# Aceinna/gnss-ins-sim

Hardware: AMD Instinct MI355X
Metric: Monte-Carlo IMU samples integrated/sec (higher is better)
Workload: dtype f64

## Files before the change

### gnss-ins-sim_amd/csrc/ginsim_api.hip

```cpp
#include <hip/hip_runtime.h>
#include <chrono>

#include <cmath>
#include <cstdarg>
#include <cstdio>
#include <cstring>
#include <string>
#include <vector>

#include "ginsim.h"
#include "allan.hpp"
#include "comm.hpp"
#include "launch.hpp"
#include "placed.hpp"

namespace ginsim {

static thread_local std::string g_err;

void set_error(const char* fmt, ...) {
    char buf[512];
    va_list ap;
    va_start(ap, fmt);
    vsnprintf(buf, sizeof(buf), fmt, ap);
    va_end(ap);
    g_err = buf;
}

}

using namespace ginsim;

struct ginsim_ctx {
    int device;
    hipStream_t stream;
    hipEvent_t ev0, ev1;
    std::vector<hipEvent_t> pool;
    void* ws[4] = {nullptr, nullptr, nullptr, nullptr};
    size_t ws_bytes[4] = {0, 0, 0, 0};
    double* allan_host = nullptr;
    size_t allan_host_doubles = 0;
    ginsim::Comm* comm = nullptr;
    double* comm_recv = nullptr;
    ginsim_stats* comm_host = nullptr;
    hipEvent_t comm_ev[8] = {};
    bool comm_pending[8] = {};
    ginsim_stats* stat_slots = nullptr;
    hipEvent_t stat_ev[8] = {};
    bool stat_pending[8] = {};
    unsigned long long* selftest = nullptr;
};

static hipError_t scratch(ginsim_ctx* c, int slot, size_t bytes, void** out) {
    if (c->ws_bytes[slot] < bytes) {
        if (c->ws[slot]) {
            hipError_t e = hipStreamSynchronize(c->stream);
            if (e != hipSuccess) return e;
            e = hipFree(c->ws[slot]);
            if (e != hipSuccess) return e;
            c->ws[slot] = nullptr;
            c->ws_bytes[slot] = 0;
        }
        const size_t want = bytes + bytes / 4 + 4096;
        hipError_t e = hipMalloc(&c->ws[slot], want);
        if (e != hipSuccess) return e;
        c->ws_bytes[slot] = want;
    }
    *out = c->ws[slot];
    return hipSuccess;
}

#define HIP_TRY(expr)                                                                         \
    do {                                                                                      \
        hipError_t e_ = (expr);                                                               \
        if (e_ != hipSuccess) {                                                               \
            set_error("%s failed: %s (%s:%d)", #expr, hipGetErrorString(e_), __FILE__, __LINE__); \
            if (e_ == hipErrorOutOfMemory) { (void)hipGetLastError(); return GINSIM_ERR_NOMEM; } \
            return GINSIM_ERR_HIP;                                                            \
        }                                                                                     \
    } while (0)
// ... 17 lines not shown

int ginsim_abi_version(void) { return GINSIM_ABI_VERSION; }

const char* ginsim_last_error(void) { return g_err.c_str(); }

int ginsim_device_count(int* count) {
    REQUIRE(count, "device_count: NULL output");
    int n = 0;
    const hipError_t e = hipGetDeviceCount(&n);
    if (e != hipSuccess) {
        *count = 0;
        set_error("hipGetDeviceCount: %s", hipGetErrorString(e));
        return GINSIM_ERR_NODEV;
    }
    *count = n;
    return GINSIM_OK;
}

int ginsim_create(int device, ginsim_ctx** out) {
    REQUIRE(out, "create: NULL output");
    *out = nullptr;
    int n = 0;
    if (hipGetDeviceCount(&n) != hipSuccess || n < 1) {
        set_error("no HIP device visible (the engine has no CPU fallback)");
        return GINSIM_ERR_NODEV;
    }
    REQUIRE(device >= 0 && device < n, "create: device %d out of range [0,%d)", device, n);
    HIP_TRY(hipSetDevice(device));
    ginsim_ctx* c = new ginsim_ctx();
    c->device = device;
    HIP_TRY(hipStreamCreateWithFlags(&c->stream, hipStreamNonBlocking));
    HIP_TRY(hipEventCreate(&c->ev0));
    HIP_TRY(hipEventCreate(&c->ev1));
    ginsim::placed_context_created(device);
    *out = c;
    return GINSIM_OK;
}

int ginsim_destroy(ginsim_ctx* c) {
    if (!c) return GINSIM_OK;
    (void)hipSetDevice(c->device);
    (void)hipStreamSynchronize(c->stream);
    (void)hipEventDestroy(c->ev0);
    (void)hipEventDestroy(c->ev1);
    for (hipEvent_t e : c->pool)
        if (e) (void)hipEventDestroy(e);
    for (void* w : c->ws)
        if (w) (void)hipFree(w);
    for (hipEvent_t e : c->stat_ev)
        if (e) (void)hipEventDestroy(e);
    if (c->stat_slots) (void)hipHostFree(c->stat_slots);
    if (c->allan_host) (void)hipHostFree(c->allan_host);
    if (c->selftest) (void)hipFree(c->selftest);
    if (c->comm) ginsim::comm_destroy(c->comm);
    if (c->comm_recv) (void)hipFree(c->comm_recv);
    if (c->comm_host) (void)hipHostFree(c->comm_host);
    for (hipEvent_t e : c->comm_ev)
        if (e) (void)hipEventDestroy(e);
    ginsim::vib_psd_drop_plans(c->stream);
    (void)hipStreamDestroy(c->stream);
    ginsim::placed_free_owner(c->device, c);
    ginsim::placed_context_destroyed(c->device);
    delete c;
    return GINSIM_OK;
}

int ginsim_device_name(ginsim_ctx* c, char* buf, size_t cap) {
    REQUIRE(c && buf && cap > 0, "device_name: bad arguments");
    hipDeviceProp_t prop;
    HIP_TRY(hipGetDeviceProperties(&prop, c->device));
    snprintf(buf, cap, "%s (%s, %d CUs)", prop.name, prop.gcnArchName, prop.multiProcessorCount);
    return GINSIM_OK;
}

int ginsim_malloc(ginsim_ctx* c, size_t bytes, void** dptr) {
    REQUIRE(c && dptr, "malloc: bad arguments");
    HIP_TRY(hipSetDevice(c->device));
    HIP_TRY(hipMalloc(dptr, bytes ? bytes : 8));
    return GINSIM_OK;
}

int ginsim_placed_configure(ginsim_ctx* c, const ginsim_placed_options* o) {
    REQUIRE(c && o, "placed_configure: bad arguments");
    return ginsim::placed_configure(c->device, *o);
// ... 463 lines not shown
}

extern "C" {

int ginsim_aux_sensors(ginsim_ctx* c, const ginsim_aux_params* p) {
    REQUIRE(c && p, "aux_sensors: NULL argument");
    REQUIRE(p->runs >= 1 && p->n >= 0 && p->m >= 0, "aux_sensors: bad sizes");
    REQUIRE(!p->out_gps || p->ref_gps, "aux_sensors: ref_gps missing");
    REQUIRE(!p->out_mag || p->ref_mag, "aux_sensors: ref_mag missing");
    REQUIRE(p->n <= 0xFFFFFFFFll && p->m <= 0xFFFFFFFFll, "aux_sensors: sample index exceeds the RNG counter");
    REQUIRE((double)p->n * (double)p->runs < 5.0e11 && (double)p->m * (double)p->runs < 5.0e11, "aux_sensors: too many elements");
    HIP_TRY(hipSetDevice(c->device));
    HIP_TRY(launch_aux(*p, c->stream));
    return GINSIM_OK;
}

int ginsim_magcal_run(ginsim_ctx* c, const ginsim_magcal_params* p) {
    REQUIRE(c && p, "magcal_run: NULL argument");
    REQUIRE(p->runs >= 1, "magcal_run: runs=%lld must be >= 1", (long long)p->runs);
    REQUIRE(p->n >= 1 && p->n <= 0xFFFFFFFFll, "magcal_run: n must lie in 1 .. the 32-bit sample counter of the RNG");
    REQUIRE(p->runs <= (int64_t)0x7FFFFFFF * 64, "magcal_run: too many runs for one launch");
    REQUIRE(p->in_mag || p->ref_mag, "magcal_run: neither ref_mag (generated form) nor in_mag (given form)");
    REQUIRE(p->out_si && p->out_hi, "magcal_run: out_si / out_hi missing");
    for (int a = 0; a < 3; ++a) {
        const long long s0 = (long long)p->seg[2 * a], s1 = (long long)p->seg[2 * a + 1];
        REQUIRE(s0 >= 0 && s1 <= (long long)p->n, "magcal_run: range %c [%lld, %lld) is outside [0, %lld]", "xyz"[a], s0, s1, (long long)p->n);
        REQUIRE(s0 < s1, "magcal_run: range %c [%lld, %lld) is empty", "xyz"[a], s0, s1);
    }
    HIP_TRY(hipSetDevice(c->device));
    HIP_TRY(launch_magcal(*p, c->stream));
    return GINSIM_OK;
}

int ginsim_end_stats(ginsim_ctx* c, const double* end_err, int64_t runs, ginsim_stats* host_out) {
    REQUIRE(c && end_err && host_out && runs >= 1, "end_stats: bad arguments");
    HIP_TRY(hipSetDevice(c->device));
    void* ws = nullptr;
    HIP_TRY(scratch(c, 0, stats_scratch_bytes(runs), &ws));
    HIP_TRY(launch_end_stats(end_err, runs, ws, c->stream));
    const char* res = reinterpret_cast<char*>(ws) + stats_scratch_bytes(runs) - sizeof(ginsim_stats);
    HIP_TRY(hipMemcpyAsync(host_out, res, sizeof(ginsim_stats), hipMemcpyDeviceToHost, c->stream));
    HIP_TRY(hipStreamSynchronize(c->stream));
    return GINSIM_OK;
}

int ginsim_end_stats_begin(ginsim_ctx* c, const double* end_err, int64_t runs, int32_t slot) {
    REQUIRE(c && end_err && runs >= 1 && slot >= 0 && slot < 8, "end_stats_begin: bad arguments");
    REQUIRE(!c->stat_pending[slot], "end_stats_begin: slot %d is still pending (call ginsim_end_stats_finish first)", slot);
    HIP_TRY(hipSetDevice(c->device));
    if (!c->stat_slots) HIP_TRY(hipHostMalloc(reinterpret_cast<void**>(&c->stat_slots), 8 * sizeof(ginsim_stats), hipHostMallocDefault));
    if (!c->stat_ev[slot]) HIP_TRY(hipEventCreateWithFlags(&c->stat_ev[slot], hipEventDisableTiming));
    void* ws = nullptr;
    HIP_TRY(scratch(c, 0, stats_scratch_bytes(runs), &ws));
    HIP_TRY(launch_end_stats(end_err, runs, ws, c->stream));
    const char* res = reinterpret_cast<char*>(ws) + stats_scratch_bytes(runs) - sizeof(ginsim_stats);
    HIP_TRY(hipMemcpyAsync(&c->stat_slots[slot], res, sizeof(ginsim_stats), hipMemcpyDeviceToHost, c->stream));
    HIP_TRY(hipEventRecord(c->stat_ev[slot], c->stream));
    c->stat_pending[slot] = true;
    return GINSIM_OK;
}

int ginsim_end_stats_finish(ginsim_ctx* c, int32_t slot, ginsim_stats* host_out) {
    REQUIRE(c && host_out && slot >= 0 && slot < 8, "end_stats_finish: bad arguments");
    REQUIRE(c->stat_pending[slot], "end_stats_finish: nothing was begun in slot %d", slot);
    HIP_TRY(hipEventSynchronize(c->stat_ev[slot]));
    *host_out = c->stat_slots[slot];
    c->stat_pending[slot] = false;
    return GINSIM_OK;
}

int ginsim_comm_unique_id(unsigned char* id) {
    REQUIRE(id, "comm_unique_id: NULL output");
    const char* err = comm_unique_id(id);
    if (err) { set_error("comm_unique_id: %s", err); return GINSIM_ERR_HIP; }
    return GINSIM_OK;
}

int ginsim_comm_init(ginsim_ctx* c, int32_t nranks, int32_t rank, const unsigned char* id) {
    REQUIRE(c && id && nranks >= 1 && rank >= 0 && rank < nranks, "comm_init: bad arguments");
    REQUIRE(!c->comm, "comm_init: this context already has a communicator");
    HIP_TRY(hipSetDevice(c->device));
    const size_t bytes = sizeof(ginsim_stats) * 8 * (size_t)nranks;
    hipError_t e = hipMalloc(reinterpret_cast<void**>(&c->comm_recv), bytes);
    if (e == hipSuccess) e = hipHostMalloc(reinterpret_cast<void**>(&c->comm_host), bytes, hipHostMallocDefault);
    const char* err = e == hipSuccess ? comm_create(nranks, rank, id, &c->comm) : nullptr;
    if (e != hipSuccess || err) {
        if (c->comm_recv) { (void)hipFree(c->comm_recv); c->comm_recv = nullptr; }
        if (c->comm_host) { (void)hipHostFree(c->comm_host); c->comm_host = nullptr; }
        c->comm = nullptr;
// ... 44 lines not shown
    return launch_vib_psd(c->device, c->stream, amp, period, runs, run_offset, seed, sensor, halve_per_run, ws, out);
}

int ginsim_comm_query(ginsim_ctx* c, int32_t* nranks, int32_t* rank, int32_t* device) {
    REQUIRE(c && nranks && rank && device, "comm_query: bad arguments");
    REQUIRE(c->comm, "comm_query: no communicator (ginsim_comm_init)");
    int n = -1, r = -1, d = -1;
    const char* err = comm_query(c->comm, &n, &r, &d);
    if (err) { set_error("comm_query: %s", err); return GINSIM_ERR_HIP; }
    *nranks = n; *rank = r; *device = d;
    return GINSIM_OK;
}

int ginsim_comm_destroy(ginsim_ctx* c) {
    REQUIRE(c, "comm_destroy: NULL context");
    if (!c->comm) return GINSIM_OK;
    HIP_TRY(hipSetDevice(c->device));
    HIP_TRY(hipStreamSynchronize(c->stream));
    comm_destroy(c->comm);
    c->comm = nullptr;
    if (c->comm_recv) { (void)hipFree(c->comm_recv); c->comm_recv = nullptr; }
    if (c->comm_host) { (void)hipHostFree(c->comm_host); c->comm_host = nullptr; }
    for (bool& p : c->comm_pending) p = false;
    return GINSIM_OK;
}

int ginsim_end_stats_all_begin(ginsim_ctx* c, const double* end_err, int64_t runs, int32_t slot) {
    REQUIRE(c && runs >= 0 && (runs == 0 || end_err) && slot >= 0 && slot < 8, "end_stats_all_begin: bad arguments");
    REQUIRE(c->comm && c->comm_recv && c->comm_host, "end_stats_all_begin: no communicator (ginsim_comm_init)");
    REQUIRE(!c->comm_pending[slot], "end_stats_all_begin: slot %d is still pending (call ginsim_end_stats_all_finish first)", slot);
    HIP_TRY(hipSetDevice(c->device));
    if (!c->comm_ev[slot]) HIP_TRY(hipEventCreateWithFlags(&c->comm_ev[slot], hipEventDisableTiming));
    const int nranks = comm_nranks(c->comm);
    void* ws = nullptr;
    const size_t wb = stats_scratch_bytes(runs > 0 ? runs : 1);
    HIP_TRY(scratch(c, 0, wb, &ws));
    double* rec = reinterpret_cast<double*>(reinterpret_cast<char*>(ws) + wb - sizeof(ginsim_stats));
    if (runs > 0) HIP_TRY(launch_end_stats(end_err, runs, ws, c->stream));
    else HIP_TRY(hipMemsetAsync(rec, 0, sizeof(ginsim_stats), c->stream));
    double* recv = c->comm_recv + (size_t)slot * nranks * (sizeof(ginsim_stats) / sizeof(double));
    const char* err = comm_allgather_f64(c->comm, rec, recv, sizeof(ginsim_stats) / sizeof(double), c->stream);
    if (err) { set_error("end_stats_all_begin: %s", err); return GINSIM_ERR_HIP; }
    HIP_TRY(hipMemcpyAsync(c->comm_host + (size_t)slot * nranks, recv, sizeof(ginsim_stats) * nranks, hipMemcpyDeviceToHost, c->stream));
    HIP_TRY(hipEventRecord(c->comm_ev[slot], c->stream));
    c->comm_pending[slot] = true;
    return GINSIM_OK;
}

int ginsim_end_stats_all_finish(ginsim_ctx* c, int32_t slot, ginsim_stats* merged) {
    REQUIRE(c && merged && slot >= 0 && slot < 8, "end_stats_all_finish: bad arguments");
    REQUIRE(c->comm && c->comm_pending[slot], "end_stats_all_finish: nothing was begun in slot %d", slot);
    HIP_TRY(hipEventSynchronize(c->comm_ev[slot]));
    c->comm_pending[slot] = false;
    const int nranks = comm_nranks(c->comm);
    std::vector<ginsim_stats> parts;
    for (int r = 0; r < nranks; ++r) {
        const ginsim_stats& p = c->comm_host[(size_t)slot * nranks + r];
        if (p.count > 0) parts.push_back(p);
    }
    memset(merged, 0, sizeof(*merged));
    if (!parts.empty()) stats_merge_host(parts.data(), (int)parts.size(), merged);
    return GINSIM_OK;
}

int ginsim_process_stats(ginsim_ctx* c, const double* traj, const double* ref, int64_t n, int64_t runs, int64_t first_sample,
                         int32_t pos_ned, double* host_out) {
    REQUIRE(c && traj && ref && host_out, "process_stats: NULL argument");
    REQUIRE(n >= 1 && runs >= 1 && first_sample >= 0 && first_sample < n, "process_stats: bad sizes");
    HIP_TRY(hipSetDevice(c->device));
    void* ws = nullptr;
    const size_t bytes = sizeof(double) * 27 * (size_t)runs;
    HIP_TRY(scratch(c, 2, bytes, &ws));
// ... 451 lines not shown
```

### gnss-ins-sim_amd/csrc/launch.hpp

```cpp
#pragma once
#include <hip/hip_runtime.h>
#include <stdint.h>
#include <stdlib.h>
#include "ginsim.h"

namespace ginsim {

void set_error(const char* fmt, ...);

hipError_t launch_mc(const ginsim_mc_params& p, hipStream_t stream, char* name, size_t cap, double* proc_about);
int mc_variant(const ginsim_mc_params& p);

hipError_t launch_mc_f32(const ginsim_mc_params& p, float* truth32, hipStream_t stream, char* name, size_t cap);
size_t mc_f32_truth_bytes(const ginsim_mc_params& p);
int mc_variant_f32(const ginsim_mc_params& p);

bool series_path_applies(const ginsim_mc_params& p);
int series_pass_b(const ginsim_mc_params& p);
int64_t series_chunks(const ginsim_mc_params& p, int32_t* L_out);
hipError_t launch_series(const ginsim_mc_params& p, double* carry, hipStream_t stream);

hipError_t launch_incl(const ginsim_mc_params& p, const ginsim_incl_params& b, hipStream_t stream, char* name, size_t cap);
int incl_variant(const ginsim_mc_params& p);

// ... 4 lines not shown
hipError_t launch_loose_aided(const ginsim_mc_params& p, const ginsim_loose_params& b, const int64_t* stamp, const int32_t* visible,
                              hipStream_t stream, char* name, size_t cap);

hipError_t launch_loose_cons(const ginsim_mc_params& p, const ginsim_loose_params& b, const ginsim_loose_cons_params& c, const int64_t* stamp,
                             const int32_t* visible, const int64_t* samples, hipStream_t stream, char* name, size_t cap);

hipError_t launch_aux(const ginsim_aux_params& p, hipStream_t s);

hipError_t launch_magcal(const ginsim_magcal_params& p, hipStream_t s);

size_t vib_psd_scratch_bytes(int64_t period, int64_t runs);
int launch_vib_psd(int device, hipStream_t stream, const double* amp, int64_t period, int64_t runs, uint64_t run_offset, uint64_t seed,
                   int sensor, int halve, void* scratch, double* out);
void vib_psd_drop_plans(hipStream_t stream);

hipError_t launch_rng_probe(uint64_t seed, uint64_t run, uint32_t stream, int64_t count, double* z0, double* z1,
                            uint32_t* words, hipStream_t stream_h);
hipError_t launch_normal_transform(const uint32_t* words, int64_t count, double* z0, double* z1, hipStream_t s);

hipError_t launch_aos_to_soa(const double* src, double* dst, int64_t R, int64_t n, int C, hipStream_t s);
hipError_t launch_runs_to_series(const double* in, double* out, int C, int64_t n, int64_t R, hipStream_t s);
hipError_t launch_gather_runs(const double* series, int C, int64_t n, int64_t runs, const int64_t* ids, int nsel,
                              double* out, hipStream_t s);
hipError_t launch_gather_series(const double* series, int C, int64_t n, const int64_t* ids, int nsel, double* out, hipStream_t s);
hipError_t launch_gather_runs_f32(const float* series, int C, int64_t n, int64_t runs, const int64_t* ids, int nsel,
                                  double* out, hipStream_t s);

hipError_t launch_pattern_fill(void* p, uint64_t words, uint32_t tag, hipStream_t s);
hipError_t launch_pattern_check(const void* p, uint64_t words, uint32_t tag, unsigned long long* out, hipStream_t s);
hipError_t launch_digest(const void* p, uint64_t words, unsigned long long* out, hipStream_t s);

size_t stats_scratch_bytes(int64_t runs);
int stats_blocks(int64_t runs);
hipError_t launch_end_stats(const double* end_err, int64_t runs, void* scratch, hipStream_t s);
void stats_merge_host(const ginsim_stats* parts, int nparts, ginsim_stats* out);
hipError_t launch_process_stats(const double* traj, const double* ref, int64_t n, int64_t runs, int64_t j0, int pos_ned,
                                int run_major, double* out, hipStream_t s);
hipError_t launch_process_stats_f32(const float* traj, const double* ref, int64_t n, int64_t runs, int64_t j0, int pos_ned,
                                    int run_major, double* out, const double* origin, int64_t n_ini, uint64_t ini_first, hipStream_t s);

size_t error_curve_scratch_bytes(const void* traj, int64_t runs, int64_t m);
hipError_t launch_error_curve(const double* traj, const double* ref, int64_t n, int64_t runs, const int64_t* samples, int64_t m,
                              int pos_ned, void* scratch, hipStream_t s);
hipError_t launch_error_curve_f32(const float* traj, const double* ref, int64_t n, int64_t runs, const int64_t* samples, int64_t m,
                                  int pos_ned, void* scratch, const double* origin, int64_t n_ini, uint64_t ini_first, hipStream_t s);
void curve_merge_host(const double* parts, int nparts, int64_t m, double* out);

inline int split_policy() {
    static const int v = [] { const char* e = getenv("GINSIM_SPLIT"); return e ? atoi(e) : -1; }();
    return v;
}

inline bool any_vibration(const ginsim_mc_params& p) { return p.vib_accel.type != GINSIM_VIB_NONE || p.vib_gyro.type != GINSIM_VIB_NONE; }
inline bool any_psd_vibration(const ginsim_mc_params& p) { return p.vib_accel.type == GINSIM_VIB_PSD || p.vib_gyro.type == GINSIM_VIB_PSD; }

inline bool any_white_drift(const ginsim_mc_params& p) {
    bool f = false;
    for (int k = 0; k < 3; ++k)
        f = f || p.accel.white_drift[k] || p.gyro.white_drift[k] || p.accel.bias[k] != 0.0 || p.gyro.bias[k] != 0.0;
    return f;
}

}
```

### gnss-ins-sim_amd/csrc/mc_kernel.hip

```cpp
#include <hip/hip_runtime.h>
#include <stdio.h>
#include <stdlib.h>
#include <type_traits>
#include "ginsim.h"
#include "ins_math.hpp"
#include "philox.hpp"
#include "device_once.hpp"
#include "sensor_synth.hpp"
#include "nav.hpp"
#include "launch.hpp"

namespace ginsim {

constexpr int kWave = 64;


template <int RF, int ALGOS, bool GIVEN, bool WD, int PS = 0, bool VIB = false>
__global__ void __launch_bounds__(256, 2) mc_kernel(const ginsim_mc_params a, const double* __restrict__ proc_about) {
    static_assert(PS == 0 || (!GIVEN && (ALGOS == GINSIM_ALGO_FREE || ALGOS == GINSIM_ALGO_ODO)), "process statistics: one algorithm, generate mode");
    static_assert(!VIB || (!GIVEN && WD), "vibration: generate mode, general sensor model");
    const int64_t r = (int64_t)blockIdx.x * blockDim.x + threadIdx.x;
    uint64_t* trace = nullptr;
    if (a.wave_trace && (threadIdx.x & 63) == 0) {
        trace = a.wave_trace + 4 * (((int64_t)blockIdx.x * blockDim.x + threadIdx.x) >> 6);
// ... 131 lines not shown
    if (PS) ps.store(a.out_proc[FREE ? 0 : 1], runs, r, (double)(n - (a.proc_first > 0 ? a.proc_first : 0)), about());
    if (trace) trace[3] = __builtin_amdgcn_s_memtime();
}

template <int RF, bool NED>
__global__ void proc_shift_kernel(const ginsim_mc_params a, double* __restrict__ about) {
    const double* ini = a.ini + 10 * (a.ini_first < (uint64_t)a.n_ini ? a.ini_first : 0);
    Nav z;
    nav_init<RF>(z, ini, a.ini_has_g);
    const double t[9] = {a.ref_nav[0], a.ref_nav[1], a.ref_nav[2], a.ref_nav[3], a.ref_nav[4], a.ref_nav[5],
                         a.ref_nav[6], a.ref_nav[7], a.ref_nav[8]};
    double e[9];
    Proc<0>::error<NED>(z, t, e);
    for (int c = 0; c < 9; ++c) about[c] = e[c];
}

constexpr int kSplitRuns = 256;
#ifndef GINSIM_SPLIT_TILE
#define GINSIM_SPLIT_TILE 6
#endif
constexpr int kSplitTile = GINSIM_SPLIT_TILE;
constexpr int kSplitStep = 12 * 4;
constexpr size_t kSplitRing = (size_t)2 * kSplitTile * kSplitStep * kSplitRuns;
constexpr size_t kSplitLds = kSplitRing > 100 * 1024 ? kSplitRing : 100 * 1024;

struct SplitInputs {
    double truth[2][ginsim::kSplitTile][8];
};
typedef const SplitInputs __attribute__((address_space(3))) * split_inputs_ptr;

#ifdef GINSIM_STEP_TIMING
constexpr int kTimingGroups = 1024;
__device__ unsigned long long g_step_timing[kTimingGroups][2];
#define GINSIM_TIMING(...) __VA_ARGS__
#else
#define GINSIM_TIMING(...)
#endif

template <int RF, int ALGOS, bool WD, int PROD = 1, bool KEEP = true, bool VIB = false>
__global__ void __launch_bounds__(256 * (1 + PROD)) mc_kernel_split(const ginsim_mc_params a_in) {
    static_assert(!VIB || WD, "vibration: general sensor model");
    constexpr int kSplitTile = VIB ? 4 : ginsim::kSplitTile;
    ginsim_mc_params a = a_in;
    if (!KEEP) {
        a.out_accel = a.out_gyro = a.out_odo = nullptr;
        a.out_traj[0] = a.out_traj[1] = nullptr;
    }
    extern __shared__ float zring[];
    constexpr bool FREE = (ALGOS & GINSIM_ALGO_FREE) != 0;
    constexpr bool ODO = (ALGOS & GINSIM_ALGO_ODO) != 0;
    constexpr int kStepFloats = (VIB ? 18 : 12) * kSplitRuns;
    const int lane = threadIdx.x & (kSplitRuns - 1);
    const bool producer = threadIdx.x >= kSplitRuns;
    const int pgroup = __builtin_amdgcn_readfirstlane((int)(threadIdx.x >> 8)) - 1;
    const int64_t r = (int64_t)blockIdx.x * kSplitRuns + lane;
    const bool active = r < a.runs;
    const int64_t n = a.n, runs = a.runs, plane = n * runs;
    const bool keep_last = a.out_accel || a.out_gyro || a.out_odo;
    const int64_t n_noise = keep_last ? n : n - 1;
    const int64_t ntiles = (n_noise + kSplitTile - 1) / kSplitTile;
    const uint64_t grun = a.run_offset + (uint64_t)r;
    const RngKey key{(uint32_t)a.seed, (uint32_t)(a.seed >> 32), (uint32_t)grun, (uint32_t)(grun >> 32)};
    MathConsts mk;
    mk.init<(ALGOS != (GINSIM_ALGO_FREE | GINSIM_ALGO_ODO))>();
    __shared__ uint32_t ntab[kNormalLdsWords];
    const NormalTables tab = fill_normal_tables(ntab, threadIdx.x, blockDim.x);
    static_assert(kSplitTile <= ginsim::kSplitTile, "SplitInputs::truth is sized by the longer tile");
    constexpr bool STAGED = PROD == 2;
    __shared__ SplitInputs in;
    const bool need_odo = ODO || a.out_odo;
    __syncthreads();


    if (producer) {
        const int sl = (int)threadIdx.x - kSplitRuns;
        for (int64_t i = 0; i <= ntiles; ++i) {
            if (STAGED && i < ntiles && sl < 8 * kSplitTile) {
                const int t = sl >> 3, c = sl & 7;
                const int64_t j = i * kSplitTile + t;
                if (j < n_noise) {
                    double v = 0.0;
                    if (c < 3) v = a.ref_accel[3 * j + c];
                    else if (c < 6) v = a.ref_gyro[3 * j + (c - 3)];
                    else if (c == 6 && need_odo) v = a.ref_odo[j];
                    in.truth[i & 1][t][c] = v;
                }
            }
            if (i < ntiles && active) {
                float* stage = zring + (i & 1) * (kSplitTile * kStepFloats);
#pragma unroll
                for (int t = 0; t < kSplitTile; ++t) {
                    const int64_t j = i * kSplitTile + t;
                    if (j < n_noise && (PROD == 1 || (t % PROD) == pgroup)) {
                        float z0[6], z1[6];
                        normal_pairs_f32<S_ACC_D_XY, 6>(key, (uint32_t)j, z0, z1, tab);
                        float* zb = stage + t * kStepFloats + lane;
#pragma unroll
                        for (int k = 0; k < 6; ++k) {
                            zb[(2 * k) * kSplitRuns] = z0[k];
                            zb[(2 * k + 1) * kSplitRuns] = z1[k];
                        }
                        if (VIB) {
                            const params_ptr kv = kernarg_params();
                            if (kv->vib_accel.type == GINSIM_VIB_RANDOM) {
                                float v0[2], v1[2];
                                normal_pairs_f32<S_ACC_VIB_XY, 2>(key, (uint32_t)j, v0, v1, tab);
                                zb[12 * kSplitRuns] = v0[0]; zb[13 * kSplitRuns] = v1[0]; zb[14 * kSplitRuns] = v0[1];
                            }
                            if (kv->vib_gyro.type == GINSIM_VIB_RANDOM) {
                                float v0[2], v1[2];
                                normal_pairs_f32<S_GYR_VIB_XY, 2>(key, (uint32_t)j, v0, v1, tab);
                                zb[15 * kSplitRuns] = v0[0]; zb[16 * kSplitRuns] = v1[0]; zb[17 * kSplitRuns] = v0[1];
                            }
                        }
                    }
                }
            }
            __syncthreads();
        }
        return;
    }

    const double dt = 1.0 / a.fs;
    const uint64_t call = a.ini_first + (uint64_t)r;
    const double* ini = a.ini + 10 * ((active && call < (uint64_t)a.n_ini) ? call : 0);
    Nav fi, od;
    if (FREE) nav_init<RF>(fi, ini, a.ini_has_g);
    if (ODO) nav_init<RF>(od, ini, a.ini_has_g);
    Vec3 da{0.0, 0.0, 0.0}, dg{0.0, 0.0, 0.0};
    Vec3 vpa{0.0, 0.0, 0.0}, vpg{0.0, 0.0, 0.0};
    if (VIB) {
        vpa = vibration_phase<S_ACC_VIB_PHASE>(&kernarg_params()->vib_accel, key);
        vpg = vibration_phase<S_GYR_VIB_PHASE>(&kernarg_params()->vib_gyro, key);
    }
    if (active) {
        if (FREE && a.out_traj[0]) store9(a.out_traj[0], plane, r, fi);
        if (ODO && a.out_traj[1]) store9(a.out_traj[1], plane, r, od);
    }
    GINSIM_TIMING(uint64_t tm_in = 0, tm_step = 0;)
    for (int64_t i = 0; i <= ntiles; ++i) {
        if (i >= 1 && active) {
            const float* stage = zring + ((i - 1) & 1) * (kSplitTile * kStepFloats);
#pragma unroll 1
            for (int t = 0; t < kSplitTile; ++t) {
                const int64_t j = (i - 1) * kSplitTile + t;
                if (j >= n_noise) break;
                const int64_t off = j * runs + r;
                const bool last = (j == n - 1);
                GINSIM_TIMING(const uint64_t tm0 = __builtin_amdgcn_s_memtime();)
                Vec3 cur_a, cur_g;
                ModelBatch ma{}, mg{};
                const double __attribute__((address_space(3))) * tr = nullptr;
                if constexpr (STAGED) {
                    split_inputs_ptr q = (split_inputs_ptr)&in;
                    asm volatile("" : "+v"(q));
                    tr = q->truth[(i - 1) & 1][t];
                    cur_a = Vec3{tr[0], tr[1], tr[2]};
                    cur_g = Vec3{tr[3], tr[4], tr[5]};
                    const params_ptr kp = kernarg_params();
                    ma = load_model(&kp->accel);
                    mg = load_model(&kp->gyro);
                    asm volatile("" :: "s"(ma.gm_a[0]), "s"(ma.gm_a[1]), "s"(ma.gm_a[2]), "s"(ma.gm_b[0]), "s"(ma.gm_b[1]), "s"(ma.gm_b[2]),
                                 "s"(ma.white[0]), "s"(ma.white[1]), "s"(ma.white[2]), "s"(mg.gm_a[0]), "s"(mg.gm_a[1]), "s"(mg.gm_a[2]),
                                 "s"(mg.gm_b[0]), "s"(mg.gm_b[1]), "s"(mg.gm_b[2]), "s"(mg.white[0]), "s"(mg.white[1]), "s"(mg.white[2]));
                } else {
                    cur_a = load3(as_uniform(a.ref_accel), j);
                    cur_g = load3(as_uniform(a.ref_gyro), j);
                }
                const float* zb = stage + t * kStepFloats + lane;
                double p0[6], p1[6];
#pragma unroll
                for (int k = 0; k < 6; ++k) {
// ... 18 lines not shown
                    double va[3] = {0.0, 0.0, 0.0}, vg[3] = {0.0, 0.0, 0.0};
                    if (kv->vib_accel.type == GINSIM_VIB_RANDOM) {
                        va[0] = (double)zb[12 * kSplitRuns]; va[1] = (double)zb[13 * kSplitRuns]; va[2] = (double)zb[14 * kSplitRuns];
                    }
                    if (kv->vib_gyro.type == GINSIM_VIB_RANDOM) {
                        vg[0] = (double)zb[15 * kSplitRuns]; vg[1] = (double)zb[16 * kSplitRuns]; vg[2] = (double)zb[17 * kSplitRuns];
                    }
                    acc = vibration_term(acc, &kv->vib_accel, va[0], va[1], va[2], (uint32_t)j, vpa);
                    gyr = vibration_term(gyr, &kv->vib_gyro, vg[0], vg[1], vg[2], (uint32_t)j, vpg);
                }
                if (a.out_accel) store3(a.out_accel, plane, off, acc);
                if (a.out_gyro) store3(a.out_gyro, plane, off, gyr);
                double odo = 0.0;
                if (need_odo) {
                    double z0, z1;
                    normal_pair(key, S_ODO, (uint32_t)j, z0, z1, tab);
                    const params_ptr kq = kernarg_params();
                    odo = kq->odo_scale * (STAGED ? tr[6] : as_uniform(a.ref_odo)[j]) + kq->odo_stdv * z0;
                    if (a.out_odo) a.out_odo[off] = odo;
                }
                if (last) break;
                const bool resync = ((j + 1) & (kTrigResync - 1)) == 0;
                if (FREE) {
                    nav_step<RF, false>(fi, gyr, acc, 0.0, dt, a.earth_rot, resync, mk);
                    if (a.out_traj[0]) store9(a.out_traj[0], plane, off + runs, fi);
                }
                if (ODO) {
                    nav_step<RF, true>(od, gyr, acc, odo, dt, a.earth_rot, resync, mk);
                    if (a.out_traj[1]) store9(a.out_traj[1], plane, off + runs, od);
                }
                GINSIM_TIMING(tm_step += __builtin_amdgcn_s_memtime() - tm0;)
            }
        }
        __syncthreads();
    }
    GINSIM_TIMING(
        if (threadIdx.x == 0 && blockIdx.x < kTimingGroups) {
            unsigned long long* q = g_step_timing[blockIdx.x];
            q[0] = tm_in; q[1] = tm_step;
        })
    if (active) {
        if (FREE && a.out_end[0]) store_end(a.out_end[0], runs, r, fi);
        if (ODO && a.out_end[1]) store_end(a.out_end[1], runs, r, od);
        if (RF == 0) {
            if (FREE && a.out_end_ned[0]) store_end_ned(a.out_end_ned[0], runs, r, fi);
            if (ODO && a.out_end_ned[1]) store_end_ned(a.out_end_ned[1], runs, r, od);
        }
    }
}

constexpr int kBlock = 256;
constexpr size_t kLdsPerCu = 160 * 1024;

int mc_variant(const ginsim_mc_params& p) {
    if (any_psd_vibration(p)) return 0;
    if (any_vibration(p)) {
        const char* env = getenv("GINSIM_SPLIT_VIB");
        return (env ? atoi(env) : 1) != 0 && split_policy() != 0 && p.algo_mask == GINSIM_ALGO_FREE && !p.given_sensors && p.block_threads == 0 &&
               !p.wave_trace && p.n >= 2 && !(p.out_proc[0] || p.out_proc[1]) && (p.runs + kWave - 1) / kWave <= 1024;
    }
    if (!(p.algo_mask & GINSIM_ALGO_FREE) || p.given_sensors || p.block_threads != 0 || p.wave_trace || p.n < 2) return 0;
    if (p.out_proc[0] || p.out_proc[1]) return 0;
    const int pol = split_policy();
    if (pol >= 0) return pol != 0;
    if (p.algo_mask == GINSIM_ALGO_FREE && p.ref_frame == 1) return 1;
    return (p.runs + kWave - 1) / kWave <= 1024 ? 1 : 0;
}

#define GINSIM_NAME_OR(fmt, ...)                         \
    if (name) {                                          \
        snprintf(name, cap, fmt, __VA_ARGS__);           \
        return hipSuccess;                               \
// ... 128 lines not shown
    }
    constexpr bool kSimpleFits = !(RF == 0 && ALGOS == (GINSIM_ALGO_FREE | GINSIM_ALGO_ODO));
    const bool proc = p.out_proc[0] || p.out_proc[1];
    const bool general_ps = proc && getenv("GINSIM_PS_GENERAL") != nullptr;
    if (any_white_drift(p) || any_vibration(p) || !kSimpleFits || (proc && p.ref_frame == 0 && p.proc_pos_ned) || general_ps)
        return launch3<RF, ALGOS, true>(p, stream, name, cap, about);
    if constexpr (kSimpleFits) return launch3<RF, ALGOS, false>(p, stream, name, cap, about);
    return hipErrorInvalidValue;
}

template <int RF>
static hipError_t launch1(const ginsim_mc_params& p, hipStream_t stream, char* name, size_t cap, double* about) {
    switch (p.algo_mask) {
        case 0: return launch2<RF, 0>(p, stream, name, cap, about);
        case GINSIM_ALGO_FREE: return launch2<RF, GINSIM_ALGO_FREE>(p, stream, name, cap, about);
        case GINSIM_ALGO_ODO: return launch2<RF, GINSIM_ALGO_ODO>(p, stream, name, cap, about);
        default: return launch2<RF, GINSIM_ALGO_FREE | GINSIM_ALGO_ODO>(p, stream, name, cap, about);
    }
}

hipError_t launch_mc(const ginsim_mc_params& p, hipStream_t stream, char* name, size_t cap, double* about) {
    return p.ref_frame == 1 ? launch1<1>(p, stream, name, cap, about) : launch1<0>(p, stream, name, cap, about);
}

}

#ifdef GINSIM_STEP_TIMING
extern "C" int ginsim_step_timing(unsigned long long* out, int groups) {
    if (groups > ginsim::kTimingGroups) groups = ginsim::kTimingGroups;
    if (hipDeviceSynchronize() != hipSuccess) return -1;
    if (hipMemcpyFromSymbol(out, HIP_SYMBOL(ginsim::g_step_timing), sizeof(unsigned long long) * 2 * groups) != hipSuccess) return -1;
    return groups;
}
#endif
```

### gnss-ins-sim_amd/csrc/stats.hip

```cpp
#include <hip/hip_runtime.h>
#include "ginsim.h"
#include "fastmath.hpp"
#include "ins_math.hpp"
#include "moments.hpp"
#include "launch.hpp"

namespace ginsim {

constexpr int kStatBlock = 256;

__device__ __forceinline__ double shift_of(const double* x) {
    const double k = x[0];
    return __builtin_isfinite(k) ? k : 0.0;
}

__global__ void __launch_bounds__(kStatBlock) stats_partial_kernel(const double* __restrict__ e, int64_t runs,
                                                                   Mom* __restrict__ partial) {
    const int comp = blockIdx.y;
    const double* x = e + (int64_t)comp * runs;
    const double k = shift_of(x);
    Mom m{0.0, 0.0, 0.0, 0.0};
    for (int64_t r = (int64_t)blockIdx.x * kStatBlock + threadIdx.x; r < runs; r += (int64_t)gridDim.x * kStatBlock) {
        const double v = x[r] - k;
        m.n += 1.0;
// ... 4 lines not shown
        } else {
            m.mean += v;
            m.m2 = __builtin_nan("");
        }
        m.mx = nan_max(fabs(x[r]), m.mx);
    }
#pragma unroll
    for (int mask = 32; mask >= 1; mask >>= 1) m = merge(m, shfl_xor(m, mask));
    __shared__ Mom wave_part[kStatBlock / 64];
    if ((threadIdx.x & 63) == 0) wave_part[threadIdx.x >> 6] = m;
    __syncthreads();
    if (threadIdx.x == 0) {
        Mom t = wave_part[0];
        for (int w = 1; w < kStatBlock / 64; ++w) t = merge(t, wave_part[w]);
        partial[comp * gridDim.x + blockIdx.x] = t;
    }
}

__global__ void stats_final_kernel(const Mom* __restrict__ partial, int blocks, const double* __restrict__ e, int64_t runs,
                                   ginsim_stats* __restrict__ out) {
    const int c = blockIdx.x;
    Mom t{0.0, 0.0, 0.0, 0.0};
    for (int b = threadIdx.x; b < blocks; b += 64) t = merge(t, partial[c * blocks + b]);
#pragma unroll
    for (int mask = 32; mask >= 1; mask >>= 1) t = merge(t, shfl_xor(t, mask));
    if (threadIdx.x == 0) {
        if (c == 0) out->count = t.n;
        out->mean[c] = shift_of(e + (int64_t)c * runs) + t.mean;
        out->m2[c] = t.m2;
        out->maxabs[c] = t.mx;
    }
}

constexpr int kSeg = 4;

template <typename T>
__global__ void __launch_bounds__(64 * kSeg) process_stats_kernel(const T* __restrict__ traj, const double* __restrict__ ref,
                                                                 int64_t n, int64_t runs, int64_t j0, int pos_ned,
                                                                 int run_major, double* __restrict__ out, const ProcOrigin org) {
    __shared__ Mom part[kSeg][9][64];
    const int lane = threadIdx.x & 63, seg = threadIdx.x >> 6;
    const int64_t r = (int64_t)blockIdx.x * 64 + lane;
    const bool active = r < runs;
    const int64_t plane = n * runs;
    const uniform_ref truth = (uniform_ref)(uintptr_t)ref;
    const int64_t len = n - j0, per = (len + kSeg - 1) / kSeg;
    const int64_t jb = j0 + seg * per, je = (jb + per < n) ? jb + per : n;
    double mean[9], m2[9], mx[9];
#pragma unroll
    for (int c = 0; c < 9; ++c) { mean[c] = 0.0; m2[c] = 0.0; mx[c] = 0.0; }
    double cnt = 0.0;
    double o3[3] = {0.0, 0.0, 0.0};
    if (org.table && active) {
        const uint64_t call = org.ini_first + (uint64_t)r;
        const double* row = org.table + 3 * (call < (uint64_t)org.n_ini ? call : 0);
        o3[0] = row[0]; o3[1] = row[1]; o3[2] = row[2];
    }
    auto error = [&](int64_t j, double (&e)[9]) {
        double x[9], t[9];
#pragma unroll
        for (int c = 0; c < 9; ++c) { x[c] = (double)traj[c * plane + j * runs + r]; t[c] = truth[9 * j + c]; }
        x[3] += o3[0]; x[4] += o3[1]; x[5] += o3[2];
        sample_error(x, t, pos_ned, e);
    };
    if (active) {
        for (int64_t j = jb; j < je; ++j) {
// ... 41 lines not shown
                out[(r * 3 + 0) * 9 + c] = t.mx;
                out[(r * 3 + 1) * 9 + c] = t.mean;
                out[(r * 3 + 2) * 9 + c] = sd;
            } else {
                out[(0 * 9 + c) * runs + r] = t.mx;
                out[(1 * 9 + c) * runs + r] = t.mean;
                out[(2 * 9 + c) * runs + r] = sd;
            }
        }
    }
}

hipError_t launch_process_stats(const double* traj, const double* ref, int64_t n, int64_t runs, int64_t j0, int pos_ned,
                                int run_major, double* out, hipStream_t s) {
    hipLaunchKernelGGL((process_stats_kernel<double>), dim3((unsigned)((runs + 63) / 64)), dim3(64 * kSeg), 0, s, traj, ref, n, runs, j0,
                       pos_ned, run_major, out, ProcOrigin{nullptr, 0, 0});
    return hipGetLastError();
}

hipError_t launch_process_stats_f32(const float* traj, const double* ref, int64_t n, int64_t runs, int64_t j0, int pos_ned,
                                    int run_major, double* out, const double* origin, int64_t n_ini, uint64_t ini_first, hipStream_t s) {
    hipLaunchKernelGGL((process_stats_kernel<float>), dim3((unsigned)((runs + 63) / 64)), dim3(64 * kSeg), 0, s, traj, ref, n, runs, j0,
                       pos_ned, run_major, out, ProcOrigin{origin, n_ini, ini_first});
    return hipGetLastError();
}

int stats_blocks(int64_t runs) {
    int64_t b = (runs + kStatBlock - 1) / kStatBlock;
    return (int)(b < 1 ? 1 : (b > 256 ? 256 : b));
}

size_t stats_scratch_bytes(int64_t runs) { return sizeof(Mom) * 9 * (size_t)stats_blocks(runs) + sizeof(ginsim_stats); }

hipError_t launch_end_stats(const double* end_err, int64_t runs, void* scratch, hipStream_t s) {
    const int blocks = stats_blocks(runs);
    Mom* partial = reinterpret_cast<Mom*>(scratch);
    ginsim_stats* out = reinterpret_cast<ginsim_stats*>(partial + 9 * blocks);
    hipLaunchKernelGGL(stats_partial_kernel, dim3(blocks, 9), dim3(kStatBlock), 0, s, end_err, runs, partial);
    hipLaunchKernelGGL(stats_final_kernel, dim3(9), dim3(64), 0, s, partial, blocks, end_err, runs, out);
    return hipGetLastError();
}

void stats_merge_host(const ginsim_stats* parts, int nparts, ginsim_stats* out) {
    for (int c = 0; c < 9; ++c) {
        Mom t{0.0, 0.0, 0.0, 0.0};
        for (int k = 0; k < nparts; ++k)
            t = merge(t, Mom{parts[k].count, parts[k].mean[c], parts[k].m2[c], parts[k].maxabs[c]});
        out->count = t.n;
        out->mean[c] = t.mean;
        out->m2[c] = t.m2;
        out->maxabs[c] = t.mx;
    }
}

}
```

Baseline: 53.87 billion.

## Fuse end-of-run stats into one last-block-reduce kernel writing pinned host memory

Replaces the two-kernel end-statistics reduction (partial kernel with a 9-column grid plus a final kernel) with a single kernel. Each block reduces all nine columns, and the last block to take an atomic ticket merges the partials and writes the result straight into mapped pinned host memory. This removes one launch and the device-to-host memcpy per stats call. It adds a persistent ticket counter that is reset in-kernel and a system-scope fence. It also adds step-timing barrier instrumentation that is compiled only under GINSIM_STEP_TIMING.

```diff
diff --git a/gnss-ins-sim_amd/csrc/ginsim_api.hip b/gnss-ins-sim_amd/csrc/ginsim_api.hip
--- a/gnss-ins-sim_amd/csrc/ginsim_api.hip
+++ b/gnss-ins-sim_amd/csrc/ginsim_api.hip
@@ -46,6 +46,8 @@
     hipEvent_t comm_ev[8] = {};
     bool comm_pending[8] = {};
     ginsim_stats* stat_slots = nullptr;
+    ginsim_stats* stat_slots_dev = nullptr;
+    unsigned* stat_ticket = nullptr;
     hipEvent_t stat_ev[8] = {};
     bool stat_pending[8] = {};
     unsigned long long* selftest = nullptr;
@@ -129,6 +131,8 @@
     HIP_TRY(hipStreamCreateWithFlags(&c->stream, hipStreamNonBlocking));
     HIP_TRY(hipEventCreate(&c->ev0));
     HIP_TRY(hipEventCreate(&c->ev1));
+    HIP_TRY(hipMalloc(reinterpret_cast<void**>(&c->stat_ticket), sizeof(unsigned)));
+    HIP_TRY(hipMemsetAsync(c->stat_ticket, 0, sizeof(unsigned), c->stream));
     ginsim::placed_context_created(device);
     *out = c;
     return GINSIM_OK;
@@ -147,6 +151,7 @@
     for (hipEvent_t e : c->stat_ev)
         if (e) (void)hipEventDestroy(e);
     if (c->stat_slots) (void)hipHostFree(c->stat_slots);
+    if (c->stat_ticket) (void)hipFree(c->stat_ticket);
     if (c->allan_host) (void)hipHostFree(c->allan_host);
     if (c->selftest) (void)hipFree(c->selftest);
     if (c->comm) ginsim::comm_destroy(c->comm);
@@ -676,15 +681,29 @@
     return GINSIM_OK;
 }
 
+static int end_stats_launch(ginsim_ctx* c, const double* end_err, int64_t runs, int slot, double** rec) {
+    void* ws = nullptr;
+    const size_t wb = stats_scratch_bytes(runs);
+    HIP_TRY(scratch(c, 0, wb, &ws));
+    char* res = reinterpret_cast<char*>(ws) + wb - sizeof(ginsim_stats);
+    if (rec) *rec = reinterpret_cast<double*>(res);
+    if (slot >= 0 && !c->stat_slots) {
+        HIP_TRY(hipHostMalloc(reinterpret_cast<void**>(&c->stat_slots), 9 * sizeof(ginsim_stats), hipHostMallocDefault));
+        HIP_TRY(hipHostGetDevicePointer(reinterpret_cast<void**>(&c->stat_slots_dev), c->stat_slots, 0));
+    }
+    const bool fused = stats_fused();
+    HIP_TRY(launch_end_stats(end_err, runs, ws, fused ? c->stat_ticket : nullptr, slot >= 0 ? c->stat_slots_dev + slot : nullptr, c->stream));
+    if (slot >= 0 && !fused) HIP_TRY(hipMemcpyAsync(&c->stat_slots[slot], res, sizeof(ginsim_stats), hipMemcpyDeviceToHost, c->stream));
+    return GINSIM_OK;
+}
+
 int ginsim_end_stats(ginsim_ctx* c, const double* end_err, int64_t runs, ginsim_stats* host_out) {
     REQUIRE(c && end_err && host_out && runs >= 1, "end_stats: bad arguments");
     HIP_TRY(hipSetDevice(c->device));
-    void* ws = nullptr;
-    HIP_TRY(scratch(c, 0, stats_scratch_bytes(runs), &ws));
-    HIP_TRY(launch_end_stats(end_err, runs, ws, c->stream));
-    const char* res = reinterpret_cast<char*>(ws) + stats_scratch_bytes(runs) - sizeof(ginsim_stats);
-    HIP_TRY(hipMemcpyAsync(host_out, res, sizeof(ginsim_stats), hipMemcpyDeviceToHost, c->stream));
-    HIP_TRY(hipStreamSynchronize(c->stream));
+    const int rc = end_stats_launch(c, end_err, runs, 8, nullptr);
+    if (rc != GINSIM_OK) return rc;
+    HIP_TRY(hipStreamSynchronize(c->stream));
+    *host_out = c->stat_slots[8];
     return GINSIM_OK;
 }
 
@@ -692,13 +711,9 @@
     REQUIRE(c && end_err && runs >= 1 && slot >= 0 && slot < 8, "end_stats_begin: bad arguments");
     REQUIRE(!c->stat_pending[slot], "end_stats_begin: slot %d is still pending (call ginsim_end_stats_finish first)", slot);
     HIP_TRY(hipSetDevice(c->device));
-    if (!c->stat_slots) HIP_TRY(hipHostMalloc(reinterpret_cast<void**>(&c->stat_slots), 8 * sizeof(ginsim_stats), hipHostMallocDefault));
     if (!c->stat_ev[slot]) HIP_TRY(hipEventCreateWithFlags(&c->stat_ev[slot], hipEventDisableTiming));
-    void* ws = nullptr;
-    HIP_TRY(scratch(c, 0, stats_scratch_bytes(runs), &ws));
-    HIP_TRY(launch_end_stats(end_err, runs, ws, c->stream));
-    const char* res = reinterpret_cast<char*>(ws) + stats_scratch_bytes(runs) - sizeof(ginsim_stats);
-    HIP_TRY(hipMemcpyAsync(&c->stat_slots[slot], res, sizeof(ginsim_stats), hipMemcpyDeviceToHost, c->stream));
+    const int rc = end_stats_launch(c, end_err, runs, slot, nullptr);
+    if (rc != GINSIM_OK) return rc;
     HIP_TRY(hipEventRecord(c->stat_ev[slot], c->stream));
     c->stat_pending[slot] = true;
     return GINSIM_OK;
@@ -809,12 +824,17 @@
     HIP_TRY(hipSetDevice(c->device));
     if (!c->comm_ev[slot]) HIP_TRY(hipEventCreateWithFlags(&c->comm_ev[slot], hipEventDisableTiming));
     const int nranks = comm_nranks(c->comm);
-    void* ws = nullptr;
-    const size_t wb = stats_scratch_bytes(runs > 0 ? runs : 1);
-    HIP_TRY(scratch(c, 0, wb, &ws));
-    double* rec = reinterpret_cast<double*>(reinterpret_cast<char*>(ws) + wb - sizeof(ginsim_stats));
-    if (runs > 0) HIP_TRY(launch_end_stats(end_err, runs, ws, c->stream));
-    else HIP_TRY(hipMemsetAsync(rec, 0, sizeof(ginsim_stats), c->stream));
+    double* rec = nullptr;
+    if (runs > 0) {
+        const int rc = end_stats_launch(c, end_err, runs, -1, &rec);
+        if (rc != GINSIM_OK) return rc;
+    } else {
+        void* ws = nullptr;
+        const size_t wb = stats_scratch_bytes(1);
+        HIP_TRY(scratch(c, 0, wb, &ws));
+        rec = reinterpret_cast<double*>(reinterpret_cast<char*>(ws) + wb - sizeof(ginsim_stats));
+        HIP_TRY(hipMemsetAsync(rec, 0, sizeof(ginsim_stats), c->stream));
+    }
     double* recv = c->comm_recv + (size_t)slot * nranks * (sizeof(ginsim_stats) / sizeof(double));
     const char* err = comm_allgather_f64(c->comm, rec, recv, sizeof(ginsim_stats) / sizeof(double), c->stream);
     if (err) { set_error("end_stats_all_begin: %s", err); return GINSIM_ERR_HIP; }
diff --git a/gnss-ins-sim_amd/csrc/launch.hpp b/gnss-ins-sim_amd/csrc/launch.hpp
--- a/gnss-ins-sim_amd/csrc/launch.hpp
+++ b/gnss-ins-sim_amd/csrc/launch.hpp
@@ -60,7 +60,9 @@
 
 size_t stats_scratch_bytes(int64_t runs);
 int stats_blocks(int64_t runs);
-hipError_t launch_end_stats(const double* end_err, int64_t runs, void* scratch, hipStream_t s);
+bool stats_fused();
+hipError_t launch_end_stats(const double* end_err, int64_t runs, void* scratch, unsigned* ticket, ginsim_stats* host_rec,
+                            hipStream_t s);
 void stats_merge_host(const ginsim_stats* parts, int nparts, ginsim_stats* out);
 hipError_t launch_process_stats(const double* traj, const double* ref, int64_t n, int64_t runs, int64_t j0, int pos_ned,
                                 int run_major, double* out, hipStream_t s);
diff --git a/gnss-ins-sim_amd/csrc/mc_kernel.hip b/gnss-ins-sim_amd/csrc/mc_kernel.hip
--- a/gnss-ins-sim_amd/csrc/mc_kernel.hip
+++ b/gnss-ins-sim_amd/csrc/mc_kernel.hip
@@ -187,6 +187,7 @@
 #ifdef GINSIM_STEP_TIMING
 constexpr int kTimingGroups = 1024;
 __device__ unsigned long long g_step_timing[kTimingGroups][2];
+__device__ unsigned long long g_barrier_timing[kTimingGroups][4][3];
 #define GINSIM_TIMING(...) __VA_ARGS__
 #else
 #define GINSIM_TIMING(...)
@@ -224,6 +225,7 @@
     constexpr bool STAGED = PROD == 2;
     __shared__ SplitInputs in;
     const bool need_odo = ODO || a.out_odo;
+    GINSIM_TIMING(__shared__ unsigned long long arrived[2][4 * (1 + PROD)];)
     __syncthreads();
 
 
@@ -271,6 +273,7 @@
                     }
                 }
             }
+            GINSIM_TIMING(if ((threadIdx.x & 63) == 0) arrived[i & 1][threadIdx.x >> 6] = __builtin_amdgcn_s_memtime();)
             __syncthreads();
         }
         return;
@@ -292,7 +295,7 @@
         if (FREE && a.out_traj[0]) store9(a.out_traj[0], plane, r, fi);
         if (ODO && a.out_traj[1]) store9(a.out_traj[1], plane, r, od);
     }
-    GINSIM_TIMING(uint64_t tm_in = 0, tm_step = 0;)
+    GINSIM_TIMING(uint64_t tm_in = 0, tm_step = 0, tb_wait = 0, tb_others = 0; const uint64_t tb_begin = __builtin_amdgcn_s_memtime();)
     for (int64_t i = 0; i <= ntiles; ++i) {
         if (i >= 1 && active) {
             const float* stage = zring + ((i - 1) & 1) * (kSplitTile * kStepFloats);
@@ -377,12 +380,27 @@
                 GINSIM_TIMING(tm_step += __builtin_amdgcn_s_memtime() - tm0;)
             }
         }
+        GINSIM_TIMING(const uint64_t tb0 = __builtin_amdgcn_s_memtime();
+                      if ((threadIdx.x & 63) == 0) arrived[i & 1][threadIdx.x >> 6] = tb0;)
         __syncthreads();
+        GINSIM_TIMING(
+            tb_wait += __builtin_amdgcn_s_memtime() - tb0;
+            unsigned long long all = 0, trio = 0;
+            for (int w = 0; w < 4 * (1 + PROD); ++w) {
+                const unsigned long long v = arrived[i & 1][w];
+                all = v > all ? v : all;
+                if ((w & 3) == (int)(threadIdx.x >> 6)) trio = v > trio ? v : trio;
+            }
+            tb_others += all - trio;)
     }
     GINSIM_TIMING(
         if (threadIdx.x == 0 && blockIdx.x < kTimingGroups) {
             unsigned long long* q = g_step_timing[blockIdx.x];
             q[0] = tm_in; q[1] = tm_step;
+        }
+        if ((threadIdx.x & 63) == 0 && blockIdx.x < kTimingGroups) {
+            unsigned long long* q = g_barrier_timing[blockIdx.x][threadIdx.x >> 6];
+            q[0] = __builtin_amdgcn_s_memtime() - tb_begin; q[1] = tb_wait; q[2] = tb_others;
         })
     if (active) {
         if (FREE && a.out_end[0]) store_end(a.out_end[0], runs, r, fi);
@@ -577,4 +595,11 @@
     if (hipMemcpyFromSymbol(out, HIP_SYMBOL(ginsim::g_step_timing), sizeof(unsigned long long) * 2 * groups) != hipSuccess) return -1;
     return groups;
 }
+
+extern "C" int ginsim_barrier_timing(unsigned long long* out, int groups) {
+    if (groups > ginsim::kTimingGroups) groups = ginsim::kTimingGroups;
+    if (hipDeviceSynchronize() != hipSuccess) return -1;
+    if (hipMemcpyFromSymbol(out, HIP_SYMBOL(ginsim::g_barrier_timing), sizeof(unsigned long long) * 12 * groups) != hipSuccess) return -1;
+    return groups;
+}
 #endif
diff --git a/gnss-ins-sim_amd/csrc/stats.hip b/gnss-ins-sim_amd/csrc/stats.hip
--- a/gnss-ins-sim_amd/csrc/stats.hip
+++ b/gnss-ins-sim_amd/csrc/stats.hip
@@ -60,6 +60,89 @@
     }
 }
 
+template <int SEGS>
+__device__ __forceinline__ void tree_reduce(Mom (*tree)[kStatBlock]) {
+    __syncthreads();
+    for (int mask = 32; mask >= 1; mask >>= 1) {
+        for (int item = threadIdx.x; item < 9 * SEGS * mask; item += kStatBlock) {
+            const int l = item & (mask - 1), seg = item / mask;
+            Mom* p = &tree[seg / SEGS][(seg % SEGS) * 64 + l];
+            *p = merge(p[0], p[mask]);
+        }
+        __syncthreads();
+    }
+}
+
+__global__ void __launch_bounds__(kStatBlock) stats_kernel(const double* __restrict__ e, int64_t runs, Mom* partial,
+                                                           unsigned* ticket, ginsim_stats* __restrict__ out,
+                                                           ginsim_stats* __restrict__ host_out) {
+    __shared__ Mom tree[9][kStatBlock];
+    __shared__ unsigned drawn;
+    const int blocks = gridDim.x;
+    double k[9];
+    Mom m[9];
+#pragma unroll
+    for (int c = 0; c < 9; ++c) { k[c] = shift_of(e + (int64_t)c * runs); m[c] = Mom{0.0, 0.0, 0.0, 0.0}; }
+    for (int64_t r = (int64_t)blockIdx.x * kStatBlock + threadIdx.x; r < runs; r += (int64_t)blocks * kStatBlock) {
+        double x[9];
+#pragma unroll
+        for (int c = 0; c < 9; ++c) x[c] = e[(int64_t)c * runs + r];
+#pragma unroll
+        for (int c = 0; c < 9; ++c) {
+            const double v = x[c] - k[c];
+            m[c].n += 1.0;
+            if (__builtin_isfinite(v) && __builtin_isfinite(m[c].mean)) {
+                const double d = v - m[c].mean;
+                m[c].mean += d / m[c].n;
+                m[c].m2 += d * (v - m[c].mean);
+            } else {
+                m[c].mean += v;
+                m[c].m2 = __builtin_nan("");
+            }
+            m[c].mx = nan_max(fabs(x[c]), m[c].mx);
+        }
+    }
+#pragma unroll
+    for (int c = 0; c < 9; ++c) tree[c][threadIdx.x] = m[c];
+    tree_reduce<kStatBlock / 64>(tree);
+    if (threadIdx.x < 9) {
+        const int c = threadIdx.x;
+        Mom t = tree[c][0];
+        for (int w = 1; w < kStatBlock / 64; ++w) t = merge(t, tree[c][64 * w]);
+        partial[c * blocks + blockIdx.x] = t;
+        __threadfence();
+    }
+    __syncthreads();
+    if (threadIdx.x == 0) drawn = __hip_atomic_fetch_add(ticket, 1u, __ATOMIC_ACQ_REL, __HIP_MEMORY_SCOPE_AGENT);
+    __syncthreads();
+    if (drawn != (unsigned)blocks - 1u) return;
+    __threadfence();
+    for (int item = threadIdx.x; item < 9 * 64; item += kStatBlock) {
+        const int c = item >> 6, lane = item & 63;
+        Mom t{0.0, 0.0, 0.0, 0.0};
+        for (int b = lane; b < blocks; b += 64) t = merge(t, partial[c * blocks + b]);
+        tree[c][lane] = t;
+    }
+    tree_reduce<1>(tree);
+    if (threadIdx.x < 9) {
+        const int c = threadIdx.x;
+        const Mom t = tree[c][0];
+        const double mean = shift_of(e + (int64_t)c * runs) + t.mean;
+        if (c == 0) out->count = t.n;
+        out->mean[c] = mean;
+        out->m2[c] = t.m2;
+        out->maxabs[c] = t.mx;
+        if (host_out) {
+            if (c == 0) host_out->count = t.n;
+            host_out->mean[c] = mean;
+            host_out->m2[c] = t.m2;
+            host_out->maxabs[c] = t.mx;
+            __threadfence_system();
+        }
+    }
+    if (threadIdx.x == 0) __hip_atomic_store(ticket, 0u, __ATOMIC_RELAXED, __HIP_MEMORY_SCOPE_AGENT);
+}
+
 constexpr int kSeg = 4;
 
 template <typename T>
@@ -167,10 +250,20 @@
 
 size_t stats_scratch_bytes(int64_t runs) { return sizeof(Mom) * 9 * (size_t)stats_blocks(runs) + sizeof(ginsim_stats); }
 
-hipError_t launch_end_stats(const double* end_err, int64_t runs, void* scratch, hipStream_t s) {
+bool stats_fused() {
+    const char* env = getenv("GINSIM_STATS_FUSED");
+    return !(env && atoi(env) == 0);
+}
+
+hipError_t launch_end_stats(const double* end_err, int64_t runs, void* scratch, unsigned* ticket, ginsim_stats* host_rec,
+                            hipStream_t s) {
     const int blocks = stats_blocks(runs);
     Mom* partial = reinterpret_cast<Mom*>(scratch);
     ginsim_stats* out = reinterpret_cast<ginsim_stats*>(partial + 9 * blocks);
+    if (ticket) {
+        hipLaunchKernelGGL(stats_kernel, dim3(blocks), dim3(kStatBlock), 0, s, end_err, runs, partial, ticket, out, host_rec);
+        return hipGetLastError();
+    }
     hipLaunchKernelGGL(stats_partial_kernel, dim3(blocks, 9), dim3(kStatBlock), 0, s, end_err, runs, partial);
     hipLaunchKernelGGL(stats_final_kernel, dim3(9), dim3(64), 0, s, partial, blocks, end_err, runs, out);
     return hipGetLastError();
```

Result: no change. 53.57 billion (-0.5%).
